# HKU-BAL/MegaGTA

Hardware: AMD Instinct MI355X
Metric: HMM-scored node expansions/sec + SdBG-build Gk-mer/s, k=45, 100Mx150bp (higher is better)
Workload: dtype u32

## Files before the change

### megagta_amd/csrc/device_utils.hpp

```cpp
#pragma once
#include <hip/hip_runtime.h>
#include <cstdint>

namespace mgta {

constexpr int kWave = 64;

__device__ __forceinline__ int lane_id() { return threadIdx.x & 63; }
__device__ __forceinline__ int wave_id() { return threadIdx.x >> 6; }
__device__ __forceinline__ uint64_t lanemask_lt() { return (1ull << lane_id()) - 1ull; }

__device__ __forceinline__ uint32_t wave_incl_scan(uint32_t v) {
    int l = lane_id();
#pragma unroll
    for (int d = 1; d < 64; d <<= 1) {
        uint32_t t = __shfl_up(v, d, 64);
        if (l >= d) v += t;
    }
    return v;
}
__device__ __forceinline__ uint64_t wave_incl_scan64(uint64_t v) {
    int l = lane_id();
#pragma unroll
    for (int d = 1; d < 64; d <<= 1) {
// ... 72 lines not shown
    uint32_t res = scratch[w] + inc - v;
    if (total) *total = scratch[NW];
    return res;
}
template <int NT>
__device__ __forceinline__ uint64_t block_excl_scan64(uint64_t v, uint64_t *scratch, uint64_t *total) {
    constexpr int NW = NT / 64;
    uint64_t inc = wave_incl_scan64(v);
    int w = wave_id(), l = lane_id();
    __syncthreads();
    if (l == 63) scratch[w] = inc;
    __syncthreads();
    if (w == 0) {
        uint64_t x = l < NW ? scratch[l] : 0;
        uint64_t xi = wave_incl_scan64(x);
        if (l < NW) scratch[l] = xi - x;
        if (l == NW - 1) scratch[NW] = xi;
    }
    __syncthreads();
    uint64_t res = scratch[w] + inc - v;
    if (total) *total = scratch[NW];
    return res;
}

constexpr unsigned long long kChainAggregate = 1ull << 62, kChainInclusive = 2ull << 62, kChainValue = (1ull << 62) - 1ull;
constexpr uint32_t kChainSpinLimit = 1u << 19;

__device__ __forceinline__ uint32_t chain_ticket(uint32_t *ticket, uint32_t *s_slot) {
    if (threadIdx.x == 0) *s_slot = atomicAdd(ticket, 1u);
    __syncthreads();
    return wave_uniform(*s_slot);
}

__device__ __forceinline__ uint64_t chain_exclusive(unsigned long long *state, uint32_t tile, uint64_t agg, uint32_t *error) {
    const int lane = lane_id();
    if (tile == 0) {
        if (lane == 0) __hip_atomic_store(&state[0], kChainInclusive | agg, __ATOMIC_RELAXED, __HIP_MEMORY_SCOPE_AGENT);
        return 0;
    }
    if (lane == 0) __hip_atomic_store(&state[tile], kChainAggregate | agg, __ATOMIC_RELAXED, __HIP_MEMORY_SCOPE_AGENT);
    uint64_t excl = 0;
    long long base = (long long)tile - 1;
    uint32_t spins = 0;
    for (;;) {
        const long long t = base - lane;
        const unsigned long long v = t >= 0 ? __hip_atomic_load(&state[t], __ATOMIC_RELAXED, __HIP_MEMORY_SCOPE_AGENT) : kChainInclusive;
        const uint32_t flag = (uint32_t)(v >> 62);
        const uint64_t empty = __ballot(flag == 0), incl = __ballot(flag == 2);
        const int first_incl = incl ? __ffsll((long long)incl) - 1 : 64;
        const uint64_t need = first_incl >= 63 ? ~0ull : ((2ull << first_incl) - 1ull);
        if (empty & need) {
            ++spins;
            if (spins > kChainSpinLimit || ((spins & 255u) == 0 && __hip_atomic_load(error, __ATOMIC_RELAXED, __HIP_MEMORY_SCOPE_AGENT))) {
                if (lane == 0) atomicExch(error, 1u);
                break;
            }
            __builtin_amdgcn_s_sleep(16);
            continue;
        }
        excl += wave_sum64(lane <= first_incl ? (uint64_t)(v & kChainValue) : 0ull);
        if (first_incl < 64) break;
        base -= 64;
    }
    if (lane == 0) __hip_atomic_store(&state[tile], kChainInclusive | ((excl + agg) & kChainValue), __ATOMIC_RELAXED, __HIP_MEMORY_SCOPE_AGENT);
    return excl;
}

}
```

### megagta_amd/csrc/sdbg_build.hip

```cpp
#include <algorithm>
#include <cmath>
#include <cstdlib>
#include <memory>
#include <type_traits>

#include "common.hpp"
#include "device_utils.hpp"
#include "scan.hpp"
#include "segment_split.hpp"

namespace mgta {

constexpr int kDollar = 4;

template <int W>
struct Key {
    uint32_t w[W];
};

template <int W>
__device__ __forceinline__ void shl_bits(uint32_t (&x)[W], int s) {
    if (s == 0) return;
    if (s == 32) {
#pragma unroll
// ... 1648 lines not shown
            uint64_t idx = base + (uint64_t)i * 256 + threadIdx.x;
            if (idx < n && key_prefix<W>(keys[idx], T) != pre && (unsigned long long)idx < found) found = idx;
        }
        if (found != ~0ull) atomicMin(&s_end, found);
        __syncthreads();
        if (s_end != ~0ull) break;
    }
    __syncthreads();
    if (threadIdx.x == 0) big_end[blockIdx.x] = s_end == ~0ull ? n : s_end;
}

constexpr int kEmitThreads = 256;
constexpr int kEmitPerThread = 16;
constexpr int kEmitTile = kEmitThreads * kEmitPerThread;

constexpr int kRunBaseStepLog = 10;
struct RunStarts {
    uint32_t *lo;
    uint64_t *base;
};
__device__ __forceinline__ uint64_t run_full_start(const RunStarts &r, uint64_t s) {
    const uint64_t b = r.base[s >> kRunBaseStepLog];
    return b + (uint32_t)(r.lo[s] - (uint32_t)b);
}
__device__ __forceinline__ uint64_t run_length(const RunStarts &r, uint64_t s, uint64_t m, uint64_t n_items) {
    return s + 1 < m ? (uint64_t)(uint32_t)(r.lo[s + 1] - r.lo[s]) : n_items - run_full_start(r, s);
}

struct EmitChain {
    unsigned long long *state;
    uint32_t *ticket;
    uint32_t *error;
    unsigned long long *total;
};

template <int W, bool TICKET>
__global__ __launch_bounds__(kEmitThreads) void emit_compact_kernel(const Key<W> *keys, uint64_t n, int k, EmitChain chain, uint32_t n_tiles,
                                                                     RunStarts sub_start, uint8_t *sub_info) {
    __shared__ uint32_t s_cnt[kEmitPerThread * (kEmitThreads / 64)];
    __shared__ uint32_t s_scr[kEmitThreads / 64 + 1];
    __shared__ uint32_t s_tile;
    __shared__ unsigned long long s_base;
    const uint32_t tile = TICKET ? chain_ticket(chain.ticket, &s_tile) : blockIdx.x;
    uint64_t base = (uint64_t)tile * kEmitTile;
    const int lane = lane_id(), wv = wave_id();
    uint32_t headbits = 0;
    uint32_t rank_in_wave[kEmitPerThread];
    uint8_t info[kEmitPerThread];
#pragma unroll
    for (int it = 0; it < kEmitPerThread; ++it) {
        uint64_t idx = base + (uint64_t)it * kEmitThreads + threadIdx.x;
        bool head = false;
        info[it] = 0;
        if (idx < n) {
            Key<W> cur = keys[idx];
            if (idx == 0) {
                head = true;
                info[it] = head_info<W>(cur, k, true, true);
            } else
                info[it] = key_info<W>(cur, keys[idx - 1], k, head);
        }
        uint64_t bal = __ballot(head);
        rank_in_wave[it] = (uint32_t)__popcll(bal & lanemask_lt());
        headbits |= (uint32_t)head << it;
        if (lane == 0) s_cnt[it * (kEmitThreads / 64) + wv] = (uint32_t)__popcll(bal);
    }
    __syncthreads();
    uint32_t v = threadIdx.x < kEmitPerThread * (kEmitThreads / 64) ? s_cnt[threadIdx.x] : 0, tile_total = 0;
    uint32_t ex = block_excl_scan<kEmitThreads>(v, s_scr, &tile_total);
    __syncthreads();
    if (threadIdx.x < kEmitPerThread * (kEmitThreads / 64)) s_cnt[threadIdx.x] = ex;
    if (wv == 0) {
        const uint64_t before = chain_exclusive(chain.state, tile, tile_total, chain.error);
        if (lane == 0) {
            s_base = before;
            if (tile + 1 == n_tiles) *chain.total = before + tile_total;
        }
    }
    __syncthreads();
    uint64_t tb = s_base;
#pragma unroll
    for (int it = 0; it < kEmitPerThread; ++it) {
        if ((headbits >> it) & 1u) {
            uint64_t idx = base + (uint64_t)it * kEmitThreads + threadIdx.x;
            uint64_t s = tb + s_cnt[it * (kEmitThreads / 64) + wv] + rank_in_wave[it];
            sub_start.lo[s] = (uint32_t)idx;
            if ((s & ((1u << kRunBaseStepLog) - 1)) == 0) sub_start.base[s >> kRunBaseStepLog] = idx;
            sub_info[s] = info[it];
        }
    }
}

constexpr int kInfoRounds = 8;
constexpr int kInfoTile = kEmitTile * kInfoRounds;
template <bool TICKET>
__global__ __launch_bounds__(kEmitThreads) void emit_compact_info_kernel(const uint8_t *info_in, uint64_t n, EmitChain chain, uint32_t n_tiles,
                                                                          RunStarts sub_start, uint8_t *sub_info) {
    static_assert(kEmitPerThread == 16, "one 16-byte load per lane and round");
    static_assert(kInfoRounds == 8 && kEmitTile <= 65535, "round counts are scanned as 2 x 4 fields of 16 bits");
    __shared__ uint64_t s_scr[kEmitThreads / 64 + 1];
    __shared__ uint32_t s_tile;
    __shared__ unsigned long long s_base;
    __shared__ uint16_t s_off[kEmitTile];
    __shared__ uint8_t s_inf[kEmitTile];
    const uint32_t tile = TICKET ? chain_ticket(chain.ticket, &s_tile) : blockIdx.x;
    const uint64_t base = (uint64_t)tile * kInfoTile;
    const uint32_t mine = threadIdx.x * kEmitPerThread;
    uint4 v[kInfoRounds];
#pragma unroll
    for (int r = 0; r < kInfoRounds; ++r) {
        const uint64_t idx0 = base + (uint64_t)r * kEmitTile + mine;
        v[r] = make_uint4(0, 0, 0, 0);
        if (idx0 < n) v[r] = *reinterpret_cast<const uint4 *>(info_in + idx0);
    }
    uint32_t headbits[kInfoRounds];
    uint64_t packed[2] = {0, 0};
#pragma unroll
    for (int r = 0; r < kInfoRounds; ++r) {
        const uint64_t idx0 = base + (uint64_t)r * kEmitTile + mine;
        const uint32_t left = idx0 < n ? (uint32_t)(n - idx0 < (uint64_t)kEmitPerThread ? n - idx0 : (uint64_t)kEmitPerThread) : 0u;
        const uint32_t wd[4] = {v[r].x, v[r].y, v[r].z, v[r].w};
        uint32_t hb = 0;
#pragma unroll
        for (int b = 0; b < kEmitPerThread; ++b) hb |= (uint32_t)(((wd[b >> 2] >> (8 * (b & 3))) & 7u) != (uint32_t)kInfoNoHead) << b;
        headbits[r] = hb & ((1u << left) - 1u);
        packed[r >> 2] |= (uint64_t)__popc(headbits[r]) << (16 * (r & 3));
    }
    uint64_t ex[2], tot[2];
    ex[0] = block_excl_scan64<kEmitThreads>(packed[0], s_scr, &tot[0]);
    ex[1] = block_excl_scan64<kEmitThreads>(packed[1], s_scr, &tot[1]);
    uint32_t round_total[kInfoRounds], round_first[kInfoRounds], tile_total = 0;
#pragma unroll
    for (int r = 0; r < kInfoRounds; ++r) {
        round_total[r] = (uint32_t)(tot[r >> 2] >> (16 * (r & 3))) & 0xFFFFu;
        round_first[r] = tile_total;
        tile_total += round_total[r];
    }
    if (wave_id() == 0) {
        const uint64_t before = chain_exclusive(chain.state, tile, tile_total, chain.error);
        if (lane_id() == 0) {
            s_base = before;
            if (tile + 1 == n_tiles) *chain.total = before + tile_total;
        }
    }
    uint64_t tb = 0;
#pragma unroll
    for (int r = 0; r < kInfoRounds; ++r) {
        if (round_total[r] == 0) continue;
        const uint32_t wd[4] = {v[r].x, v[r].y, v[r].z, v[r].w};
        uint32_t q = (uint32_t)(ex[r >> 2] >> (16 * (r & 3))) & 0xFFFFu;
#pragma unroll
        for (int b = 0; b < kEmitPerThread; ++b) {
            if ((headbits[r] >> b) & 1u) {
                s_off[q] = (uint16_t)(mine + (uint32_t)b);
                s_inf[q] = (uint8_t)((wd[b >> 2] >> (8 * (b & 3))) & 255u);
                ++q;
            }
        }
        __syncthreads();
        tb = s_base;
        const uint64_t out0 = tb + round_first[r], pos0 = base + (uint64_t)r * kEmitTile;
        for (uint32_t i = threadIdx.x; i < round_total[r]; i += kEmitThreads) {
            const uint64_t s = out0 + i, idx = pos0 + s_off[i];
            sub_start.lo[s] = (uint32_t)idx;
            if ((s & ((1u << kRunBaseStepLog) - 1)) == 0) sub_start.base[s >> kRunBaseStepLog] = idx;
            sub_info[s] = s_inf[i];
        }
        __syncthreads();
    }
}

__global__ __launch_bounds__(256) void emit_check_kernel(const uint32_t *lo, const uint8_t *info, const uint32_t *lo_ref, const uint8_t *info_ref, uint64_t m,
                                                         uint32_t *bad) {
    for (uint64_t s = (uint64_t)blockIdx.x * 256 + threadIdx.x; s < m; s += (uint64_t)gridDim.x * 256) {
        if (lo[s] != lo_ref[s]) atomicAdd(&bad[0], 1u);
        if (info[s] != info_ref[s]) atomicAdd(&bad[1], 1u);
    }
}

template <int W>
__global__ __launch_bounds__(256) void emit_info_range_kernel(const Key<W> *keys, uint64_t n, int k, const uint64_t *start, const uint64_t *end, int stride,
                                                              uint8_t *key_info_out) {
    const uint64_t first = start[(uint64_t)blockIdx.x * stride] & ~kSegInOther;
    uint64_t last = end[(uint64_t)blockIdx.x * stride];
    if (last > n) last = n;
    for (uint64_t i = first + threadIdx.x; i < last; i += 256) {
        const Key<W> cur = keys[i];
        bool head = true;
        const uint8_t info = i == 0 ? head_info<W>(cur, k, true, true) : key_info<W>(cur, keys[i - 1], k, head);
        key_info_out[i] = head ? info : kInfoNoHead;
    }
}

constexpr int kDecideThreads = 256;
constexpr int kDecidePerThread = 4;
constexpr int kDecideTile = kDecideThreads * kDecidePerThread;
constexpr int kDecideHalo = 32;

__device__ __forceinline__ bool run_suppressed(int a, int b, int has_a, int has_b) {
    return (a == kDollar && ((has_b >> b) & 1)) || (b == kDollar && ((has_a >> a) & 1));
}

// ... 53 lines not shown
            ne++;
            nl += count > 254;
            nt += tip;
        }
        rec[s] = r;
    }
    ne = wave_sum(ne); nl = wave_sum(nl); nt = wave_sum(nt);
    if (lane_id() == 0) { s_e[wave_id()] = ne; s_l[wave_id()] = nl; s_t[wave_id()] = nt; }
    __syncthreads();
    if (threadIdx.x == 0) {
        uint32_t e = 0, l = 0, t = 0;
        for (int w = 0; w < kDecideThreads / 64; ++w) { e += s_e[w]; l += s_l[w]; t += s_t[w]; }
        cnt_e[blockIdx.x] = e; cnt_l[blockIdx.x] = l; cnt_t[blockIdx.x] = t;
    }
}

template <int W>
__global__ __launch_bounds__(kDecideThreads) void emit_write_kernel(const Key<W> *keys, RunStarts sub_start, const uint8_t *sub_info, const uint16_t *rec,
                                                                     uint64_t m, uint64_t n_items, const uint64_t *base_e,
                                                                     const uint64_t *base_l, const uint64_t *base_t, int words_per_tip,
                                                                     uint32_t b_lo, uint16_t *out_rec, uint16_t *out_large,
                                                                     uint32_t *out_tips, int64_t *bucket_first ) {
    __shared__ uint64_t s_scr[kDecideThreads / 64 + 1];
    uint64_t s0 = (uint64_t)blockIdx.x * kDecideTile + (uint64_t)threadIdx.x * kDecidePerThread;
    uint16_t r[kDecidePerThread];
    uint64_t packed = 0;
    uint32_t cnts[kDecidePerThread];
    for (int q = 0; q < kDecidePerThread; ++q) {
        uint64_t s = s0 + q;
        r[q] = 0xFFFF; cnts[q] = 0;
        if (s < m) {
            r[q] = rec[s];
            if (r[q] != 0xFFFF) {
                uint64_t run = run_length(sub_start, s, m, n_items);
                cnts[q] = run > 65535 ? 65535u : (uint32_t)run;
                packed += 1ull + ((uint64_t)(cnts[q] > 254) << 20) + ((uint64_t)((r[q] >> 5) & 1) << 40);
            }
        }
    }
    uint64_t ex = block_excl_scan64<kDecideThreads>(packed, s_scr, nullptr);
    uint64_t ie = base_e[blockIdx.x] + (ex & 0xFFFFF), il = base_l[blockIdx.x] + ((ex >> 20) & 0xFFFFF),
             it = base_t[blockIdx.x] + (ex >> 40);
    for (int q = 0; q < kDecidePerThread; ++q) {
        uint64_t s = s0 + q;
        if (s >= m) break;
        const bool is_tip = r[q] != 0xFFFF && ((r[q] >> 5) & 1);
        const bool bucket_head = (sub_info[s] & 128) != 0;
        const uint64_t first_item = (is_tip || bucket_head) ? run_full_start(sub_start, s) : 0;
        if (bucket_head) {
            uint32_t bucket = keys[first_item].w[0] >> 16;
            int64_t *bf = bucket_first + (uint64_t)(bucket - b_lo) * 3;
            bf[0] = (int64_t)ie; bf[1] = (int64_t)il; bf[2] = (int64_t)it;
        }
        if (r[q] != 0xFFFF) {
            out_rec[ie++] = r[q];
            if (cnts[q] > 254) out_large[il++] = (uint16_t)cnts[q];
            if ((r[q] >> 5) & 1) {
                for (int j = 0; j < words_per_tip; ++j) out_tips[it * words_per_tip + j] = keys[first_item].w[j];
                it++;
            }
        }
    }
}

}
#include "sdbg_solid.hpp"
namespace mgta {

static std::vector<Digit> low_digit_plan(int k, int W, int T) {
    std::vector<Digit> plan;
    int pad = 32 * W - 2 * k - 4, top = 32 * W - T;
    if (top > 0) plan.push_back(Digit{0, std::min(4, top)});
    for (int pos = 4 + pad; pos < top; pos += 8) plan.push_back(Digit{pos, std::min(8, top - pos)});
    return plan;
}

template <class T>
static T *pool_get(mgta_ctx *ctx, int slot, uint64_t bytes) {
    if ((int)ctx->pool.size() < S_NUM) ctx->pool.resize(S_NUM);
    DevBuf &b = ctx->pool[slot];
    if (b.bytes < bytes || !b.p) {
        b.release();
        b.alloc(bytes + bytes / 8, &ctx->live_bytes, &ctx->peak_bytes);
    }
    return b.as<T>();
}
static uint64_t pool_bytes(const mgta_ctx *ctx) {
    uint64_t t = 0;
    for (const DevBuf &b : ctx->pool) t += b.bytes;
    return t;
}

struct SortModes {
    int bias = 1, side = 1, fused = 1, wide = 1, emit_fused = 1;
    static SortModes from_env() {
        const char *bias = getenv("MGTA_SORT_BIAS"), *side = getenv("MGTA_SORT_SIDE"), *fused = getenv("MGTA_SORT_FUSED"), *wide = getenv("MGTA_SORT_WIDE");
        const char *emit_fused = getenv("MGTA_EMIT_FUSED");
        return SortModes{bias ? atoi(bias) : 1, side ? atoi(side) : 1, fused ? atoi(fused) : 1, wide ? atoi(wide) : 1, emit_fused ? atoi(emit_fused) : 1};
    }
};

static double avg_segment_len(uint64_t n_items, int p, double prefix_frac) { return (double)n_items / std::max(1.0, std::pow(256.0, p) * prefix_frac); }
static double avg_segment_len_bits(uint64_t n_items, int bits, double prefix_frac) { return (double)n_items / std::max(1.0, std::pow(2.0, bits) * prefix_frac); }
constexpr int kMaxTop = 4;
struct TopPlan {
    int P = 0, skip = 0;
    uint32_t bias = 0;
    double frac = 1.0;
    int width[kMaxTop] = {8, 8, 8, 8};
    int key_bits() const { int t = 0; for (int i = 0; i < P; ++i) t += width[i]; return t; }
    int T() const { return key_bits() + skip; }
    int n_wide() const { int c = 0; for (int i = 0; i < P; ++i) c += width[i] > 8; return c; }
    int max_width() const { int m = 8; for (int i = 0; i < P; ++i) m = std::max(m, width[i]); return m; }
    bool same_digits(const TopPlan &o) const {
        bool same = P == o.P && skip == o.skip && bias == o.bias;
        for (int i = 0; same && i < P; ++i) same = width[i] == o.width[i];
        return same;
    }
    Digit pass_digit(int W, int i) const {
        int below = skip;
        for (int j = 0; j <= i; ++j) below += width[j];
        return Digit{32 * W - below, width[i], bias};
    }
    double avg_segment(uint64_t n_items) const { return avg_segment_len_bits(n_items, key_bits(), frac); }
};
static TopPlan choose_top_plan(const mgta_ctx *ctx, uint64_t n_items, int max_top, double prefix_frac, uint32_t b_lo = 0, uint32_t b_hi = 0,
                               int mode = 0) {
    TopPlan plain;
    plain.frac = prefix_frac;
    if (ctx && ctx->force_full_lsd) return plain;
    while (plain.P < max_top && avg_segment_len(n_items, plain.P, prefix_frac) > (plain.P >= 3 ? 700.0 : 256.0)) ++plain.P;
// ... 713 lines not shown
            sa.side = nullptr;
        }
        S.ms_gen += t_ph.stop();
    }

    Key<W> *sort_keys(const SortJob<W> &job) {
        t_ph.start();
        Key<W> *sorted = device_sort(ctx, job, &log, &sorted_info);
        if (sorted) S.ms_sort += t_ph.stop();
        return sorted;
    }

    int drop_sentinels(Pass &p) {
        if (!p.closed_form || ((k + 1) & 1)) return MGTA_OK;
        unsigned long long n_sent = 0;
        MGTA_HIP_CHECK(hipMemcpy(&n_sent, d_sentinel, 8, hipMemcpyDeviceToHost));
        if (n_sent >= p.n_items) { set_error("internal: %llu sentinel keys among %llu items", n_sent, (unsigned long long)p.n_items); return MGTA_EINTERNAL; }
        p.n_items -= n_sent;
        S.n_items -= (int64_t)n_sent;
        return MGTA_OK;
    }

    int emit(Pass &p, const Key<W> *sorted, Key<W> *scratch_keys) {
        const uint64_t n_items = p.n_items;
        t_ph.start();
        char *scratch = reinterpret_cast<char *>(scratch_keys);
        uint64_t e_tiles = (n_items + kEmitTile - 1) / kEmitTile;
        uint64_t *d_scan_tmp = pool_get<uint64_t>(ctx, S_SCAN_TMP, scan_tmp_elems(std::max<uint64_t>(std::max(n_blocks, e_tiles), n_items / kDecideTile + 1)) * 8);
        if (e_tiles > 0xFFFFFFFFull) { set_error("too many emit tiles"); return MGTA_EUNSUPPORTED; }
        unsigned long long *d_chain = pool_get<unsigned long long>(ctx, S_TILE_BASE, (e_tiles + 4) * 8);
        RunStarts sub_start;
        sub_start.lo = reinterpret_cast<uint32_t *>(scratch);
        uint16_t *rec = reinterpret_cast<uint16_t *>(scratch + n_items * 4);
        uint8_t *info = reinterpret_cast<uint8_t *>(scratch + n_items * 6);
        sub_start.base = reinterpret_cast<uint64_t *>(scratch + ((n_items * 7 + 7) & ~7ull));
        auto compact = [&](const uint8_t *key_info, RunStarts st, uint8_t *st_info, uint64_t *m_out) {
            unsigned long long chain_out[3] = {0, 0, 0};
            const uint64_t tiles = key_info ? (n_items + kInfoTile - 1) / kInfoTile : e_tiles;
            EmitChain chain;
            chain.state = d_chain; chain.total = d_chain + tiles;
            chain.ticket = reinterpret_cast<uint32_t *>(d_chain + tiles + 1); chain.error = reinterpret_cast<uint32_t *>(d_chain + tiles + 2);
            for (int attempt = 0; attempt < 2; ++attempt) {
                MGTA_HIP_CHECK(hipMemsetAsync(d_chain, 0, (tiles + 4) * 8, stream));
                const bool ticket = !(attempt == 0 && !ctx->force_full_lsd);
                const dim3 grid((unsigned)tiles), block(kEmitThreads);
                if (key_info && !ticket)
                    hipLaunchKernelGGL((emit_compact_info_kernel<false>), grid, block, 0, stream, key_info, n_items, chain, (uint32_t)tiles, st, st_info);
                else if (key_info)
                    hipLaunchKernelGGL((emit_compact_info_kernel<true>), grid, block, 0, stream, key_info, n_items, chain, (uint32_t)tiles, st, st_info);
                else if (!ticket)
                    hipLaunchKernelGGL((emit_compact_kernel<W, false>), grid, block, 0, stream, sorted, n_items, k, chain, (uint32_t)tiles, st, st_info);
                else
                    hipLaunchKernelGGL((emit_compact_kernel<W, true>), grid, block, 0, stream, sorted, n_items, k, chain, (uint32_t)tiles, st, st_info);
                MGTA_HIP_CHECK(hipMemcpyAsync(chain_out, d_chain + tiles, 24, hipMemcpyDeviceToHost, stream));
                MGTA_HIP_CHECK(hipStreamSynchronize(stream));
                if ((uint32_t)chain_out[2] == 0) break;
            }
            if ((uint32_t)chain_out[2] != 0) { set_error("internal: chained scan of the emitter timed out"); return MGTA_EINTERNAL; }
            *m_out = chain_out[0];
            return MGTA_OK;
        };
        uint64_t m = 0;
        if (int rc = compact(sorted_info, sub_start, info, &m)) return rc;
        if (sorted_info) {
            ctx->emit_fused_passes++;
            if (modes.emit_fused >= 2) {
                RunStarts ref;
                uint8_t *ref_info = reinterpret_cast<uint8_t *>(rec);
                char *behind = reinterpret_cast<char *>(sub_start.base + (n_items >> kRunBaseStepLog) + 1);
                ref.lo = reinterpret_cast<uint32_t *>(behind);
                ref.base = reinterpret_cast<uint64_t *>(behind + ((n_items * 4 + 7) & ~7ull));
                if ((uint64_t)(reinterpret_cast<char *>(ref.base + (n_items >> kRunBaseStepLog) + 1) - scratch) > p.key_b) {
                    set_error("internal: no room to check the emitter's info bytes");
                    return MGTA_EINTERNAL;
                }
                uint64_t m_ref = 0;
                if (int rc = compact(nullptr, ref, ref_info, &m_ref)) return rc;
                uint32_t *d_bad = reinterpret_cast<uint32_t *>(pool_get<uint64_t>(ctx, S_SMALL, 4096) + 320);
                uint32_t bad[2] = {0, 0};
                MGTA_HIP_CHECK(hipMemsetAsync(d_bad, 0, 8, stream));
                const uint64_t m_min = std::min(m, m_ref);
                if (m_min > 0) {
                    const unsigned grid = (unsigned)std::min<uint64_t>((m_min + 255) / 256, (uint64_t)ctx->num_cus * 16);
                    hipLaunchKernelGGL(emit_check_kernel, dim3(grid), dim3(256), 0, stream, sub_start.lo, info, ref.lo, ref_info, m_min, d_bad);
                }
                MGTA_HIP_CHECK(hipMemcpyAsync(bad, d_bad, 8, hipMemcpyDeviceToHost, stream));
                MGTA_HIP_CHECK(hipStreamSynchronize(stream));
                if (m != m_ref || bad[0] || bad[1]) {
                    set_error("internal: the info bytes of the sort give %llu runs, the keys %llu; %u starts and %u info bytes differ",
                              (unsigned long long)m, (unsigned long long)m_ref, bad[0], bad[1]);
                    return MGTA_EINTERNAL;
                }
            }
        }
        uint64_t d_tiles = (m + kDecideTile - 1) / kDecideTile;
        uint32_t *ce = pool_get<uint32_t>(ctx, S_CNT, d_tiles * 4 * 3), *cl = ce + d_tiles, *ct = cl + d_tiles;
        uint64_t *be = pool_get<uint64_t>(ctx, S_BASE, d_tiles * 8 * 3), *bl = be + d_tiles, *bt = bl + d_tiles;
        p.first = pool_get<int64_t>(ctx, S_FIRST, (uint64_t)MGTA_NUM_BUCKETS * 3 * 8);
        MGTA_HIP_CHECK(hipMemsetAsync(p.first, 0xFF, (uint64_t)p.nb() * 3 * 8, stream));
        hipLaunchKernelGGL(emit_decide_kernel, dim3((unsigned)d_tiles), dim3(kDecideThreads), 0, stream, sub_start, info, m, n_items,
                           rec, ce, cl, ct);
        exclusive_scan_u32(stream, ce, d_tiles, be, d_scan_tmp, d_tot3);
        exclusive_scan_u32(stream, cl, d_tiles, bl, d_scan_tmp, d_tot3 + 1);
        exclusive_scan_u32(stream, ct, d_tiles, bt, d_scan_tmp, d_tot3 + 2);
        uint64_t tot3[3];
        MGTA_HIP_CHECK(hipMemcpyAsync(tot3, d_tot3, 24, hipMemcpyDeviceToHost, stream));
        MGTA_HIP_CHECK(hipStreamSynchronize(stream));
        p.n_edges = tot3[0]; p.n_large = tot3[1]; p.n_tips = tot3[2];
        p.rec = pool_get<uint16_t>(ctx, S_OUT_REC, p.n_edges * 2);
        p.large = pool_get<uint16_t>(ctx, S_OUT_LARGE, p.n_large * 2);
        p.tips = pool_get<uint32_t>(ctx, S_OUT_TIPS, p.n_tips * words_per_tip * 4);
        hipLaunchKernelGGL((emit_write_kernel<W>), dim3((unsigned)d_tiles), dim3(kDecideThreads), 0, stream, sorted, sub_start, info, rec, m,
                           n_items, be, bl, bt, words_per_tip, p.b_lo, p.rec, p.large, p.tips, p.first);
        S.ms_emit += t_ph.stop();
        return MGTA_OK;
    }

    void publish_last(uint32_t lo, uint32_t hi, const void *rec, uint64_t n_rec, const void *tips, uint64_t n_tips, const void *first,
                      const void *large, uint64_t n_large) {
        ctx->last_large = large; ctx->last_n_large = n_large;
        ctx->last_rec = rec; ctx->last_n_rec = n_rec; ctx->last_bucket_lo = lo; ctx->last_bucket_hi = hi;
        ctx->last_tips = tips; ctx->last_n_tips = n_tips; ctx->last_first = first; ctx->last_k = k; ctx->last_words_per_tip = words_per_tip;
    }

    void append_to_stream(const Pass &p) {
        const uint64_t tip_b = words_per_tip * 4;
        auto ensure = [&](DevBuf &buf, uint64_t used, uint64_t add) {
            if (used + add <= buf.bytes) return;
            const double done = (double)(p.b_hi - bucket_begin) / (double)(bucket_end - bucket_begin);
            uint64_t want = (uint64_t)((double)(used + add) / std::max(done, 1e-3) * 1.1) + (1u << 20);
            want = std::max<uint64_t>(want, used + add);
            DevBuf bigger;
            bigger.alloc(want, &ctx->live_bytes, &ctx->peak_bytes);
            if (used) MGTA_HIP_CHECK(hipMemcpyAsync(bigger.p, buf.p, used, hipMemcpyDeviceToDevice, stream));
            MGTA_HIP_CHECK(hipStreamSynchronize(stream));
            buf = std::move(bigger);
        };
        ensure(ctx->acc_rec, ctx->acc_n_rec * 2, p.n_edges * 2);
        ensure(ctx->acc_tips, ctx->acc_n_tips * tip_b, p.n_tips * tip_b);
        if (ctx->acc_has_large) {
            ensure(ctx->acc_large, ctx->acc_n_large * 2, p.n_large * 2);
            if (p.n_large) MGTA_HIP_CHECK(hipMemcpyAsync(ctx->acc_large.as<char>() + ctx->acc_n_large * 2, p.large, p.n_large * 2, hipMemcpyDeviceToDevice, stream));
        }
        if (p.n_edges) MGTA_HIP_CHECK(hipMemcpyAsync(ctx->acc_rec.as<char>() + ctx->acc_n_rec * 2, p.rec, p.n_edges * 2, hipMemcpyDeviceToDevice, stream));
        if (p.n_tips) MGTA_HIP_CHECK(hipMemcpyAsync(ctx->acc_tips.as<char>() + ctx->acc_n_tips * tip_b, p.tips, p.n_tips * tip_b, hipMemcpyDeviceToDevice, stream));
        h_first.resize((size_t)p.nb() * 3);
// ... 189 lines not shown
```

Before: 10.08.

## Fuse emitter decide, scan and write into one chained-scan kernel

Replaces the emit path's three stages (a decide kernel, three exclusive scans, a host readback and sync, then a write kernel) with one kernel. That kernel decides records per tile, publishes counts through two decoupled look-back chains and writes compacted output through shared memory. Output buffers are sized up front from upper bounds (run count, dollar heads counted in the compact kernel, n_items/255), which removes the mid-pass host round trip. It also stores small run counts in the record's high byte so the write kernel can skip run_length lookups. The cost is larger allocations, spin-wait risk with a retry path, and a verification mode that runs both paths.

```diff
diff --git a/megagta_amd/csrc/device_utils.hpp b/megagta_amd/csrc/device_utils.hpp
--- a/megagta_amd/csrc/device_utils.hpp
+++ b/megagta_amd/csrc/device_utils.hpp
@@ -128,13 +128,12 @@
     return wave_uniform(*s_slot);
 }
 
-__device__ __forceinline__ uint64_t chain_exclusive(unsigned long long *state, uint32_t tile, uint64_t agg, uint32_t *error) {
+__device__ __forceinline__ void chain_publish(unsigned long long *state, uint32_t tile, uint64_t agg) {
+    if (lane_id() == 0) __hip_atomic_store(&state[tile], (tile == 0 ? kChainInclusive : kChainAggregate) | agg, __ATOMIC_RELAXED, __HIP_MEMORY_SCOPE_AGENT);
+}
+__device__ __forceinline__ uint64_t chain_look_back(unsigned long long *state, uint32_t tile, uint64_t agg, uint32_t *error) {
     const int lane = lane_id();
-    if (tile == 0) {
-        if (lane == 0) __hip_atomic_store(&state[0], kChainInclusive | agg, __ATOMIC_RELAXED, __HIP_MEMORY_SCOPE_AGENT);
-        return 0;
-    }
-    if (lane == 0) __hip_atomic_store(&state[tile], kChainAggregate | agg, __ATOMIC_RELAXED, __HIP_MEMORY_SCOPE_AGENT);
+    if (tile == 0) return 0;
     uint64_t excl = 0;
     long long base = (long long)tile - 1;
     uint32_t spins = 0;
@@ -161,5 +160,9 @@
     if (lane == 0) __hip_atomic_store(&state[tile], kChainInclusive | ((excl + agg) & kChainValue), __ATOMIC_RELAXED, __HIP_MEMORY_SCOPE_AGENT);
     return excl;
 }
+__device__ __forceinline__ uint64_t chain_exclusive(unsigned long long *state, uint32_t tile, uint64_t agg, uint32_t *error) {
+    chain_publish(state, tile, agg);
+    return chain_look_back(state, tile, agg, error);
+}
 
 }
diff --git a/megagta_amd/csrc/sdbg_build.hip b/megagta_amd/csrc/sdbg_build.hip
--- a/megagta_amd/csrc/sdbg_build.hip
+++ b/megagta_amd/csrc/sdbg_build.hip
@@ -1704,19 +1704,29 @@
     uint32_t *ticket;
     uint32_t *error;
     unsigned long long *total;
+    unsigned long long *dollar;
 };
+constexpr int kDollarSlots = 64;
+__device__ __forceinline__ void count_dollar_heads(const EmitChain &chain, uint32_t tile, uint32_t mine, uint32_t *s_sum) {
+    if (threadIdx.x == 0) *s_sum = 0;
+    __syncthreads();
+    mine = wave_sum(mine);
+    if (lane_id() == 0 && mine) atomicAdd(s_sum, mine);
+    __syncthreads();
+    if (threadIdx.x == 0 && *s_sum) atomicAdd(&chain.dollar[tile % kDollarSlots], (unsigned long long)*s_sum);
+}
 
 template <int W, bool TICKET>
 __global__ __launch_bounds__(kEmitThreads) void emit_compact_kernel(const Key<W> *keys, uint64_t n, int k, EmitChain chain, uint32_t n_tiles,
                                                                      RunStarts sub_start, uint8_t *sub_info) {
     __shared__ uint32_t s_cnt[kEmitPerThread * (kEmitThreads / 64)];
     __shared__ uint32_t s_scr[kEmitThreads / 64 + 1];
-    __shared__ uint32_t s_tile;
+    __shared__ uint32_t s_tile, s_dollar;
     __shared__ unsigned long long s_base;
     const uint32_t tile = TICKET ? chain_ticket(chain.ticket, &s_tile) : blockIdx.x;
     uint64_t base = (uint64_t)tile * kEmitTile;
     const int lane = lane_id(), wv = wave_id();
-    uint32_t headbits = 0;
+    uint32_t headbits = 0, n_dollar = 0;
     uint32_t rank_in_wave[kEmitPerThread];
     uint8_t info[kEmitPerThread];
 #pragma unroll
@@ -1759,8 +1769,10 @@
             sub_start.lo[s] = (uint32_t)idx;
             if ((s & ((1u << kRunBaseStepLog) - 1)) == 0) sub_start.base[s >> kRunBaseStepLog] = idx;
             sub_info[s] = info[it];
-        }
-    }
+            n_dollar += (info[it] & 7) == kDollar;
+        }
+    }
+    count_dollar_heads(chain, tile, n_dollar, &s_dollar);
 }
 
 constexpr int kInfoRounds = 8;
@@ -1771,7 +1783,7 @@
     static_assert(kEmitPerThread == 16, "one 16-byte load per lane and round");
     static_assert(kInfoRounds == 8 && kEmitTile <= 65535, "round counts are scanned as 2 x 4 fields of 16 bits");
     __shared__ uint64_t s_scr[kEmitThreads / 64 + 1];
-    __shared__ uint32_t s_tile;
+    __shared__ uint32_t s_tile, s_dollar;
     __shared__ unsigned long long s_base;
     __shared__ uint16_t s_off[kEmitTile];
     __shared__ uint8_t s_inf[kEmitTile];
@@ -1816,6 +1828,7 @@
         }
     }
     uint64_t tb = 0;
+    uint32_t n_dollar = 0;
 #pragma unroll
     for (int r = 0; r < kInfoRounds; ++r) {
         if (round_total[r] == 0) continue;
@@ -1836,10 +1849,13 @@
             const uint64_t s = out0 + i, idx = pos0 + s_off[i];
             sub_start.lo[s] = (uint32_t)idx;
             if ((s & ((1u << kRunBaseStepLog) - 1)) == 0) sub_start.base[s >> kRunBaseStepLog] = idx;
-            sub_info[s] = s_inf[i];
+            const uint8_t inf = s_inf[i];
+            sub_info[s] = inf;
+            n_dollar += (inf & 7) == kDollar;
         }
         __syncthreads();
     }
+    count_dollar_heads(chain, tile, n_dollar, &s_dollar);
 }
 
 __global__ __launch_bounds__(256) void emit_check_kernel(const uint32_t *lo, const uint8_t *info, const uint32_t *lo_ref, const uint8_t *info_ref, uint64_t m,
@@ -1959,8 +1975,11 @@
         if (s < m) {
             r[q] = rec[s];
             if (r[q] != 0xFFFF) {
-                uint64_t run = run_length(sub_start, s, m, n_items);
-                cnts[q] = run > 65535 ? 65535u : (uint32_t)run;
+                cnts[q] = r[q] >> 8;
+                if (cnts[q] == 255) {
+                    uint64_t run = run_length(sub_start, s, m, n_items);
+                    cnts[q] = run > 65535 ? 65535u : (uint32_t)run;
+                }
                 packed += 1ull + ((uint64_t)(cnts[q] > 254) << 20) + ((uint64_t)((r[q] >> 5) & 1) << 40);
             }
         }
@@ -1990,6 +2009,243 @@
     }
 }
 
+constexpr int kChainRounds = 8;
+constexpr int kChainTile = kDecideTile * kChainRounds;
+constexpr int kChainSlots = kChainRounds * kDecidePerThread * (kDecideThreads / 64);
+constexpr int kChainTipBits = 34;
+static_assert(kChainTipBits < 62 && kChainTile < (1 << 20), "the second chain's value, the packed tile counts");
+struct DecideChain {
+    unsigned long long *state_e, *state_lt;
+    uint32_t *ticket, *error;
+    uint64_t *totals;
+};
+
+template <int W, bool TICKET>
+__global__ __launch_bounds__(kDecideThreads, 6) void emit_decide_write_kernel(const Key<W> *keys, RunStarts sub_start, const uint8_t *sub_info, uint64_t m,
+                                                                            uint64_t n_items, DecideChain chain, uint32_t n_tiles, int words_per_tip,
+                                                                            uint32_t b_lo, uint16_t *out_rec, uint16_t *out_large, uint32_t *out_tips,
+                                                                            int64_t *bucket_first ) {
+    constexpr int NW = kDecideThreads / 64, NQ = kDecidePerThread;
+    constexpr int kChunks = (kChainTile + 2 * kDecideHalo) / 16, kChunkIters = (kChunks + kDecideThreads - 1) / kDecideThreads;
+    static_assert(NQ == 4 && kDecideHalo % 16 == 0 && kChainSlots <= kDecideThreads, "four decisions per word; 16-byte loads; one scan");
+    __shared__ uint4 s_info4[kChunks];
+    __shared__ uint16_t s_out[kChainTile];
+    __shared__ uint64_t s_cnt[kChainSlots];
+    __shared__ uint64_t s_scr[NW + 1];
+    __shared__ uint32_t s_tile;
+    __shared__ unsigned long long s_base[2];
+    const uint8_t *s_info = reinterpret_cast<const uint8_t *>(s_info4);
+    const uint32_t tile = TICKET ? chain_ticket(chain.ticket, &s_tile) : blockIdx.x;
+    const uint64_t t0 = (uint64_t)tile * kChainTile;
+    const uint32_t tid = threadIdx.x;
+    const int lane = lane_id(), wv = wave_id();
+    const uint8_t *info_t = sub_info + t0;
+    const uint32_t *lo_t = sub_start.lo + t0;
+    const int m_l = (int)(m - t0 < (1ull << 30) ? m - t0 : (1ull << 30));
+    const uint32_t n_t = (uint32_t)(m_l < kChainTile + 1 ? m_l : kChainTile + 1);
+    const int w_lo = tile ? -kDecideHalo : 0, w_hi = m_l < kChainTile + kDecideHalo ? m_l : kChainTile + kDecideHalo;
+
+    uint4 iv[kChunkIters];
+#pragma unroll
+    for (int j = 0; j < kChunkIters; ++j) {
+        const uint32_t c = (uint32_t)j * kDecideThreads + tid;
+        const int at = 16 * (int)c - kDecideHalo;
+        iv[j] = make_uint4(0, 0, 0, 0);
+        if (c < (uint32_t)kChunks && at >= w_lo && at < m_l) iv[j] = *reinterpret_cast<const uint4 *>(info_t + at);
+    }
+    uint32_t cnt2[kChainRounds][NQ / 2];
+    const bool owns_last = n_t <= (uint32_t)kChainTile && ((n_t - 1) & (kDecideThreads - 1)) == tid;
+    uint32_t last_len = 0;
+#pragma unroll
+    for (int half = 0; half < 2; ++half) {
+        uint32_t lo0[kChainRounds / 2][NQ], lo1[kChainRounds / 2][NQ];
+#pragma unroll
+        for (int r = 0; r < kChainRounds / 2; ++r)
+#pragma unroll
+            for (int q = 0; q < NQ; ++q) {
+                const uint32_t idx = (uint32_t)(((half * (kChainRounds / 2) + r) * NQ + q) * kDecideThreads) + tid;
+                lo0[r][q] = lo_t[idx < n_t - 1 ? idx : n_t - 1];
+                lo1[r][q] = lo_t[idx + 1 < n_t - 1 ? idx + 1 : n_t - 1];
+            }
+        if (half == 0) {
+#pragma unroll
+            for (int j = 0; j < kChunkIters; ++j) {
+                const uint32_t c = (uint32_t)j * kDecideThreads + tid;
+                if (c < (uint32_t)kChunks) s_info4[c] = iv[j];
+            }
+            if (owns_last) {
+                const uint64_t rest = n_items - run_full_start(sub_start, t0 + n_t - 1);
+                last_len = rest > 65535 ? 65535u : (uint32_t)rest;
+            }
+        }
+        __builtin_amdgcn_sched_barrier(0);
+#pragma unroll
+        for (int r = 0; r < kChainRounds / 2; ++r) {
+            const int rr = half * (kChainRounds / 2) + r;
+            cnt2[rr][0] = cnt2[rr][1] = 0;
+#pragma unroll
+            for (int q = 0; q < NQ; ++q) {
+                uint32_t len = lo1[r][q] - lo0[r][q];
+                if (owns_last && (uint32_t)(rr * NQ + q) == (n_t - 1) / kDecideThreads) len = last_len;
+                cnt2[rr][q >> 1] |= (len > 65535u ? 65535u : len) << (16 * (q & 1));
+            }
+            asm volatile("" : "+v"(cnt2[rr][0]), "+v"(cnt2[rr][1]));
+        }
+        __builtin_amdgcn_sched_barrier(0);
+    }
+    __syncthreads();
+
+    auto info_at = [&](int j) -> int { return (j >= w_lo && j < w_hi) ? (int)s_info[j + kDecideHalo] : (int)info_t[j]; };
+    uint32_t dec[kChainRounds];
+#pragma unroll
+    for (int r = 0; r < kChainRounds; ++r) dec[r] = ~0u;
+#pragma unroll 1
+    for (int r = 0; r < kChainRounds; ++r) {
+        uint32_t c01 = 0, c23 = 0, dr = 0;
+#pragma unroll
+        for (int rr = 0; rr < kChainRounds; ++rr)
+            if (rr == r) { c01 = cnt2[rr][0]; c23 = cnt2[rr][1]; }
+#pragma unroll
+        for (int q = 0; q < NQ; ++q) {
+            const int s = (r * NQ + q) * kDecideThreads + (int)tid;
+            const uint32_t count = ((q & 2 ? c23 : c01) >> (16 * (q & 1))) & 0xFFFFu;
+            uint32_t d = 0xFFu;
+            if (s < m_l) {
+                const int inf = info_at(s);
+                const int a = inf & 7, b = (inf >> 3) & 7;
+                int has_a = 0, has_b = 0;
+                auto collect = [&](int xi) {
+                    const int xa = xi & 7, xb = (xi >> 3) & 7;
+                    if (xa != kDollar && xb != kDollar) { has_a |= 1 << xa; has_b |= 1 << xb; }
+                };
+                collect(inf);
+                bool front_b_solid = false, front_b_dollar = false;
+                int gs = s;
+                for (int gi = inf; !(gi & 64);) {
+                    --gs; gi = info_at(gs); collect(gi);
+                    if (((gi >> 3) & 7) == b) { if ((gi & 7) != kDollar) front_b_solid = true; else front_b_dollar = true; }
+                }
+                int ge = s + 1;
+                while (ge < m_l) {
+                    const int xi = info_at(ge);
+                    if (xi & 64) break;
+                    collect(xi);
+                    ++ge;
+                }
+                if (!run_suppressed(a, b, has_a, has_b)) {
+                    const bool seen_b = front_b_solid || (front_b_dollar && !((has_b >> b) & 1));
+                    const int w = (b == kDollar) ? 0 : (seen_b ? b + 5 : b + 1);
+                    int last = 0;
+                    if (a != kDollar) {
+                        bool later = false;
+                        for (int x = s + 1; x < ge; ++x) {
+                            const int xi = info_at(x), xa = xi & 7, xb = (xi >> 3) & 7;
+                            if (xa == a && (xb != kDollar || !((has_a >> a) & 1))) later = true;
+                        }
+                        last = later ? 0 : 1;
+                    }
+                    d = (uint32_t)(w | (last << 4) | ((a == kDollar) << 5));
+                }
+            }
+            dr |= d << (8 * q);
+            const bool em = d != 0xFFu;
+            const uint64_t bal_e = __ballot(em), bal_l = __ballot(em && count > 254u), bal_t = __ballot(em && (d & 32u));
+            if (lane == 0)
+                s_cnt[(r * NQ + q) * NW + wv] = (uint64_t)__popcll(bal_e) | (uint64_t)__popcll(bal_l) << 20 | (uint64_t)__popcll(bal_t) << 40;
+        }
+#pragma unroll
+        for (int rr = 0; rr < kChainRounds; ++rr)
+            if (rr == r) dec[rr] = dr;
+    }
+    __syncthreads();
+
+    uint64_t tot = 0;
+    const uint64_t ex = block_excl_scan64<kDecideThreads>(tid < (uint32_t)kChainSlots ? s_cnt[tid] : 0ull, s_scr, &tot);
+    if (tid < (uint32_t)kChainSlots) s_cnt[tid] = ex;
+    const uint32_t te = (uint32_t)tot & 0xFFFFFu, tl = (uint32_t)(tot >> 20) & 0xFFFFFu, tt = (uint32_t)(tot >> 40);
+    const uint64_t agg_lt = (uint64_t)tl << kChainTipBits | tt;
+    if (wv == 0) chain_publish(chain.state_e, tile, te);
+    if (wv == 1) chain_publish(chain.state_lt, tile, agg_lt);
+    __syncthreads();
+
+#pragma unroll
+    for (int r = 0; r < kChainRounds; ++r)
+#pragma unroll
+        for (int q = 0; q < NQ; ++q) {
+            const uint32_t d = (dec[r] >> (8 * q)) & 0xFFu, count = (cnt2[r][q >> 1] >> (16 * (q & 1))) & 0xFFFFu;
+            const bool em = d != 0xFFu;
+            const uint64_t bal_e = __ballot(em);
+            if (em) {
+                const uint32_t at = ((uint32_t)s_cnt[(r * NQ + q) * NW + wv] & 0xFFFFFu) + (uint32_t)__popcll(bal_e & lanemask_lt());
+                s_out[at] = (uint16_t)(d | (count > 255u ? 255u : count) << 8);
+            }
+        }
+    if (wv == 0) {
+        const uint64_t before = chain_look_back(chain.state_e, tile, te, chain.error);
+        if (lane == 0) {
+            s_base[0] = before;
+            if (tile + 1 == n_tiles) chain.totals[0] = before + te;
+        }
+    }
+    if (wv == 1) {
+        const uint64_t before = chain_look_back(chain.state_lt, tile, agg_lt, chain.error);
+        if (lane == 0) {
+            s_base[1] = before;
+            if (tile + 1 == n_tiles) { chain.totals[1] = (before >> kChainTipBits) + tl; chain.totals[2] = (before & ((1ull << kChainTipBits) - 1ull)) + tt; }
+        }
+    }
+    __syncthreads();
+    const uint64_t be = s_base[0], bl = s_base[1] >> kChainTipBits, bt = s_base[1] & ((1ull << kChainTipBits) - 1ull);
+
+    {
+        uint32_t head = (uint32_t)((8u - (uint32_t)(be & 7u)) & 7u);
+        if (head > te) head = te;
+        const uint32_t n8 = (te - head) >> 3, tail0 = head + (n8 << 3);
+        if (tid < head) out_rec[be + tid] = s_out[tid];
+        for (uint32_t c = tid; c < n8; c += kDecideThreads) {
+            const uint32_t i = head + (c << 3);
+            uint4 v;
+            v.x = (uint32_t)s_out[i] | (uint32_t)s_out[i + 1] << 16; v.y = (uint32_t)s_out[i + 2] | (uint32_t)s_out[i + 3] << 16;
+            v.z = (uint32_t)s_out[i + 4] | (uint32_t)s_out[i + 5] << 16; v.w = (uint32_t)s_out[i + 6] | (uint32_t)s_out[i + 7] << 16;
+            *reinterpret_cast<uint4 *>(out_rec + be + i) = v;
+        }
+        if (tail0 + tid < te) out_rec[be + tail0 + tid] = s_out[tail0 + tid];
+    }
+
+#pragma unroll
+    for (int r = 0; r < kChainRounds; ++r)
+#pragma unroll
+        for (int q = 0; q < NQ; ++q) {
+            const int k0 = (r * NQ + q) * kDecideThreads;
+            const uint32_t d = (dec[r] >> (8 * q)) & 0xFFu, count = (cnt2[r][q >> 1] >> (16 * (q & 1))) & 0xFFFFu;
+            const bool em = d != 0xFFu, large = em && count > 254u, tip = em && (d & 32u);
+            const bool bucket_head = (int)tid < m_l - k0 && (s_info[kDecideHalo + k0 + tid] & 128) != 0;
+            if (__ballot(large || tip || bucket_head) == 0) continue;
+            const uint64_t bal_e = __ballot(em), bal_l = __ballot(large), bal_t = __ballot(tip), lt = lanemask_lt();
+            const uint64_t x = s_cnt[(r * NQ + q) * NW + wv];
+            const uint64_t ie = be + ((uint32_t)x & 0xFFFFFu) + (uint32_t)__popcll(bal_e & lt);
+            const uint64_t il = bl + ((uint32_t)(x >> 20) & 0xFFFFFu) + (uint32_t)__popcll(bal_l & lt);
+            const uint64_t it = bt + (uint32_t)(x >> 40) + (uint32_t)__popcll(bal_t & lt);
+            if (large) out_large[il] = (uint16_t)count;
+            if (tip || bucket_head) {
+                const uint64_t first_item = run_full_start(sub_start, t0 + k0 + tid);
+                if (bucket_head) {
+                    const uint32_t bucket = keys[first_item].w[0] >> 16;
+                    int64_t *bf = bucket_first + (uint64_t)(bucket - b_lo) * 3;
+                    bf[0] = (int64_t)ie; bf[1] = (int64_t)il; bf[2] = (int64_t)it;
+                }
+                if (tip)
+                    for (int j = 0; j < words_per_tip; ++j) out_tips[it * words_per_tip + j] = keys[first_item].w[j];
+            }
+        }
+}
+
+template <class T>
+__global__ __launch_bounds__(256) void emit_equal_kernel(const T *a, const T *b, uint64_t n, uint32_t *bad) {
+    for (uint64_t i = (uint64_t)blockIdx.x * 256 + threadIdx.x; i < n; i += (uint64_t)gridDim.x * 256)
+        if (a[i] != b[i]) atomicAdd(bad, 1u);
+}
+
 }
 #include "sdbg_solid.hpp"
 namespace mgta {
@@ -2019,11 +2275,12 @@
 }
 
 struct SortModes {
-    int bias = 1, side = 1, fused = 1, wide = 1, emit_fused = 1;
+    int bias = 1, side = 1, fused = 1, wide = 1, emit_fused = 1, emit_chain = 1;
     static SortModes from_env() {
         const char *bias = getenv("MGTA_SORT_BIAS"), *side = getenv("MGTA_SORT_SIDE"), *fused = getenv("MGTA_SORT_FUSED"), *wide = getenv("MGTA_SORT_WIDE");
-        const char *emit_fused = getenv("MGTA_EMIT_FUSED");
-        return SortModes{bias ? atoi(bias) : 1, side ? atoi(side) : 1, fused ? atoi(fused) : 1, wide ? atoi(wide) : 1, emit_fused ? atoi(emit_fused) : 1};
+        const char *emit_fused = getenv("MGTA_EMIT_FUSED"), *emit_chain = getenv("MGTA_EMIT_CHAIN");
+        return SortModes{bias ? atoi(bias) : 1, side ? atoi(side) : 1, fused ? atoi(fused) : 1, wide ? atoi(wide) : 1, emit_fused ? atoi(emit_fused) : 1,
+                         emit_chain ? atoi(emit_chain) : 1};
     }
 };
 
@@ -2803,16 +3060,20 @@
         RunStarts sub_start;
         sub_start.lo = reinterpret_cast<uint32_t *>(scratch);
         uint16_t *rec = reinterpret_cast<uint16_t *>(scratch + n_items * 4);
-        uint8_t *info = reinterpret_cast<uint8_t *>(scratch + n_items * 6);
-        sub_start.base = reinterpret_cast<uint64_t *>(scratch + ((n_items * 7 + 7) & ~7ull));
-        auto compact = [&](const uint8_t *key_info, RunStarts st, uint8_t *st_info, uint64_t *m_out) {
+        const uint64_t info_at = (n_items * 6 + 15) & ~15ull;
+        uint8_t *info = reinterpret_cast<uint8_t *>(scratch + info_at);
+        sub_start.base = reinterpret_cast<uint64_t *>(scratch + ((info_at + n_items + 15) & ~15ull));
+        unsigned long long *d_dollar = reinterpret_cast<unsigned long long *>(pool_get<uint64_t>(ctx, S_SMALL, 4096) + 64);
+        auto compact = [&](const uint8_t *key_info, RunStarts st, uint8_t *st_info, uint64_t *m_out, uint64_t *n_dollar_out) {
             unsigned long long chain_out[3] = {0, 0, 0};
+            unsigned long long dollar[kDollarSlots];
             const uint64_t tiles = key_info ? (n_items + kInfoTile - 1) / kInfoTile : e_tiles;
             EmitChain chain;
-            chain.state = d_chain; chain.total = d_chain + tiles;
+            chain.state = d_chain; chain.total = d_chain + tiles; chain.dollar = d_dollar;
             chain.ticket = reinterpret_cast<uint32_t *>(d_chain + tiles + 1); chain.error = reinterpret_cast<uint32_t *>(d_chain + tiles + 2);
             for (int attempt = 0; attempt < 2; ++attempt) {
                 MGTA_HIP_CHECK(hipMemsetAsync(d_chain, 0, (tiles + 4) * 8, stream));
+                MGTA_HIP_CHECK(hipMemsetAsync(d_dollar, 0, sizeof(dollar), stream));
                 const bool ticket = !(attempt == 0 && !ctx->force_full_lsd);
                 const dim3 grid((unsigned)tiles), block(kEmitThreads);
                 if (key_info && !ticket)
@@ -2824,15 +3085,18 @@
                 else
                     hipLaunchKernelGGL((emit_compact_kernel<W, true>), grid, block, 0, stream, sorted, n_items, k, chain, (uint32_t)tiles, st, st_info);
                 MGTA_HIP_CHECK(hipMemcpyAsync(chain_out, d_chain + tiles, 24, hipMemcpyDeviceToHost, stream));
+                MGTA_HIP_CHECK(hipMemcpyAsync(dollar, d_dollar, sizeof(dollar), hipMemcpyDeviceToHost, stream));
                 MGTA_HIP_CHECK(hipStreamSynchronize(stream));
                 if ((uint32_t)chain_out[2] == 0) break;
             }
             if ((uint32_t)chain_out[2] != 0) { set_error("internal: chained scan of the emitter timed out"); return MGTA_EINTERNAL; }
             *m_out = chain_out[0];
+            *n_dollar_out = 0;
+            for (unsigned long long d : dollar) *n_dollar_out += d;
             return MGTA_OK;
         };
-        uint64_t m = 0;
-        if (int rc = compact(sorted_info, sub_start, info, &m)) return rc;
+        uint64_t m = 0, n_dollar = 0;
+        if (int rc = compact(sorted_info, sub_start, info, &m, &n_dollar)) return rc;
         if (sorted_info) {
             ctx->emit_fused_passes++;
             if (modes.emit_fused >= 2) {
@@ -2845,8 +3109,10 @@
                     set_error("internal: no room to check the emitter's info bytes");
                     return MGTA_EINTERNAL;
                 }
-                uint64_t m_ref = 0;
-                if (int rc = compact(nullptr, ref, ref_info, &m_ref)) return rc;
+                uint64_t m_ref = 0, n_dollar_ref = 0;
+                if (int rc = compact(nullptr, ref, ref_info, &m_ref, &n_dollar_ref)) return rc;
+                if (n_dollar_ref != n_dollar) { set_error("internal: the info bytes of the sort give %llu runs with a = $, the keys %llu",
+                                                          (unsigned long long)n_dollar, (unsigned long long)n_dollar_ref); return MGTA_EINTERNAL; }
                 uint32_t *d_bad = reinterpret_cast<uint32_t *>(pool_get<uint64_t>(ctx, S_SMALL, 4096) + 320);
                 uint32_t bad[2] = {0, 0};
                 MGTA_HIP_CHECK(hipMemsetAsync(d_bad, 0, 8, stream));
@@ -2864,25 +3130,104 @@
                 }
             }
         }
-        uint64_t d_tiles = (m + kDecideTile - 1) / kDecideTile;
-        uint32_t *ce = pool_get<uint32_t>(ctx, S_CNT, d_tiles * 4 * 3), *cl = ce + d_tiles, *ct = cl + d_tiles;
-        uint64_t *be = pool_get<uint64_t>(ctx, S_BASE, d_tiles * 8 * 3), *bl = be + d_tiles, *bt = bl + d_tiles;
-        p.first = pool_get<int64_t>(ctx, S_FIRST, (uint64_t)MGTA_NUM_BUCKETS * 3 * 8);
-        MGTA_HIP_CHECK(hipMemsetAsync(p.first, 0xFF, (uint64_t)p.nb() * 3 * 8, stream));
-        hipLaunchKernelGGL(emit_decide_kernel, dim3((unsigned)d_tiles), dim3(kDecideThreads), 0, stream, sub_start, info, m, n_items,
-                           rec, ce, cl, ct);
-        exclusive_scan_u32(stream, ce, d_tiles, be, d_scan_tmp, d_tot3);
-        exclusive_scan_u32(stream, cl, d_tiles, bl, d_scan_tmp, d_tot3 + 1);
-        exclusive_scan_u32(stream, ct, d_tiles, bt, d_scan_tmp, d_tot3 + 2);
-        uint64_t tot3[3];
-        MGTA_HIP_CHECK(hipMemcpyAsync(tot3, d_tot3, 24, hipMemcpyDeviceToHost, stream));
-        MGTA_HIP_CHECK(hipStreamSynchronize(stream));
-        p.n_edges = tot3[0]; p.n_large = tot3[1]; p.n_tips = tot3[2];
-        p.rec = pool_get<uint16_t>(ctx, S_OUT_REC, p.n_edges * 2);
-        p.large = pool_get<uint16_t>(ctx, S_OUT_LARGE, p.n_large * 2);
-        p.tips = pool_get<uint32_t>(ctx, S_OUT_TIPS, p.n_tips * words_per_tip * 4);
-        hipLaunchKernelGGL((emit_write_kernel<W>), dim3((unsigned)d_tiles), dim3(kDecideThreads), 0, stream, sorted, sub_start, info, rec, m,
-                           n_items, be, bl, bt, words_per_tip, p.b_lo, p.rec, p.large, p.tips, p.first);
+        struct Out { uint16_t *rec = nullptr, *large = nullptr; uint32_t *tips = nullptr; int64_t *first = nullptr; uint64_t tot[3] = {0, 0, 0}; };
+        DevBuf t_rec, t_large, t_tips, t_first;
+        auto room = [&](bool pooled, int slot, DevBuf &tmp, uint64_t bytes) -> void * {
+            if (pooled) return pool_get<char>(ctx, slot, bytes);
+            tmp.alloc(bytes, &ctx->live_bytes, &ctx->peak_bytes);
+            return tmp.p;
+        };
+        const uint64_t first_b = (uint64_t)MGTA_NUM_BUCKETS * 3 * 8;
+        auto three_steps = [&](bool pooled, Out &o) -> int {
+            const uint64_t d_tiles = (m + kDecideTile - 1) / kDecideTile;
+            uint32_t *ce = pool_get<uint32_t>(ctx, S_CNT, d_tiles * 4 * 3), *cl = ce + d_tiles, *ct = cl + d_tiles;
+            uint64_t *be = pool_get<uint64_t>(ctx, S_BASE, d_tiles * 8 * 3), *bl = be + d_tiles, *bt = bl + d_tiles;
+            o.first = static_cast<int64_t *>(room(pooled, S_FIRST, t_first, first_b));
+            MGTA_HIP_CHECK(hipMemsetAsync(o.first, 0xFF, (uint64_t)p.nb() * 3 * 8, stream));
+            hipLaunchKernelGGL(emit_decide_kernel, dim3((unsigned)d_tiles), dim3(kDecideThreads), 0, stream, sub_start, info, m, n_items,
+                               rec, ce, cl, ct);
+            exclusive_scan_u32(stream, ce, d_tiles, be, d_scan_tmp, d_tot3);
+            exclusive_scan_u32(stream, cl, d_tiles, bl, d_scan_tmp, d_tot3 + 1);
+            exclusive_scan_u32(stream, ct, d_tiles, bt, d_scan_tmp, d_tot3 + 2);
+            MGTA_HIP_CHECK(hipMemcpyAsync(o.tot, d_tot3, 24, hipMemcpyDeviceToHost, stream));
+            MGTA_HIP_CHECK(hipStreamSynchronize(stream));
+            o.rec = static_cast<uint16_t *>(room(pooled, S_OUT_REC, t_rec, o.tot[0] * 2));
+            o.large = static_cast<uint16_t *>(room(pooled, S_OUT_LARGE, t_large, o.tot[1] * 2));
+            o.tips = static_cast<uint32_t *>(room(pooled, S_OUT_TIPS, t_tips, o.tot[2] * words_per_tip * 4));
+            hipLaunchKernelGGL((emit_write_kernel<W>), dim3((unsigned)d_tiles), dim3(kDecideThreads), 0, stream, sorted, sub_start, info, rec, m,
+                               n_items, be, bl, bt, words_per_tip, p.b_lo, o.rec, o.large, o.tips, o.first);
+            return MGTA_OK;
+        };
+        auto chained = [&](Out &o) -> int {
+            if ((m >> kChainTipBits) != 0 || ((n_items / 255) >> (62 - kChainTipBits)) != 0) {
+                set_error("too many runs (%llu) or keys (%llu) for the emitter's chained scan", (unsigned long long)m, (unsigned long long)n_items);
+                return MGTA_EUNSUPPORTED;
+            }
+            const uint64_t tiles = (m + kChainTile - 1) / kChainTile;
+            DecideChain dc;
+            dc.state_e = d_chain; dc.state_lt = d_chain + tiles; dc.totals = d_tot3;
+            dc.ticket = reinterpret_cast<uint32_t *>(d_chain + 2 * tiles); dc.error = reinterpret_cast<uint32_t *>(d_chain + 2 * tiles + 1);
+            o.rec = pool_get<uint16_t>(ctx, S_OUT_REC, m * 2);
+            o.large = pool_get<uint16_t>(ctx, S_OUT_LARGE, (n_items / 255 + 1) * 2);
+            o.tips = pool_get<uint32_t>(ctx, S_OUT_TIPS, n_dollar * words_per_tip * 4);
+            o.first = pool_get<int64_t>(ctx, S_FIRST, first_b);
+            unsigned long long err = 0;
+            for (int attempt = 0; attempt < 2; ++attempt) {
+                MGTA_HIP_CHECK(hipMemsetAsync(d_chain, 0, (2 * tiles + 2) * 8, stream));
+                MGTA_HIP_CHECK(hipMemsetAsync(d_tot3, 0, 24, stream));
+                MGTA_HIP_CHECK(hipMemsetAsync(o.first, 0xFF, (uint64_t)p.nb() * 3 * 8, stream));
+                const dim3 grid((unsigned)tiles), block(kDecideThreads);
+                if (attempt == 0 && !ctx->force_full_lsd)
+                    hipLaunchKernelGGL((emit_decide_write_kernel<W, false>), grid, block, 0, stream, sorted, sub_start, info, m, n_items, dc, (uint32_t)tiles,
+                                       words_per_tip, p.b_lo, o.rec, o.large, o.tips, o.first);
+                else
+                    hipLaunchKernelGGL((emit_decide_write_kernel<W, true>), grid, block, 0, stream, sorted, sub_start, info, m, n_items, dc, (uint32_t)tiles,
+                                       words_per_tip, p.b_lo, o.rec, o.large, o.tips, o.first);
+                MGTA_HIP_CHECK(hipMemcpyAsync(o.tot, d_tot3, 24, hipMemcpyDeviceToHost, stream));
+                MGTA_HIP_CHECK(hipMemcpyAsync(&err, d_chain + 2 * tiles + 1, 8, hipMemcpyDeviceToHost, stream));
+                MGTA_HIP_CHECK(hipStreamSynchronize(stream));
+                if ((uint32_t)err == 0) break;
+            }
+            if ((uint32_t)err != 0) { set_error("internal: chained scan of the emitter's records timed out"); return MGTA_EINTERNAL; }
+            if (o.tot[0] > m || o.tot[1] > n_items / 255 + 1 || o.tot[2] > n_dollar) {
+                set_error("internal: the emitter wrote %llu records, %llu large counts and %llu tips into room for %llu, %llu and %llu", (unsigned long long)o.tot[0],
+                          (unsigned long long)o.tot[1], (unsigned long long)o.tot[2], (unsigned long long)m, (unsigned long long)(n_items / 255 + 1), (unsigned long long)n_dollar);
+                return MGTA_EINTERNAL;
+            }
+            return MGTA_OK;
+        };
+        Out out, ref;
+        if (modes.emit_chain <= 0) {
+            if (int rc = three_steps(true, out)) return rc;
+        } else {
+            if (modes.emit_chain >= 2)
+                if (int rc = three_steps(false, ref)) return rc;
+            if (int rc = chained(out)) return rc;
+        }
+        if (modes.emit_chain >= 2) {
+            uint32_t *d_bad = reinterpret_cast<uint32_t *>(pool_get<uint64_t>(ctx, S_SMALL, 4096) + 320);
+            uint32_t bad[4] = {0, 0, 0, 0};
+            MGTA_HIP_CHECK(hipMemsetAsync(d_bad, 0, 16, stream));
+            const bool same_totals = out.tot[0] == ref.tot[0] && out.tot[1] == ref.tot[1] && out.tot[2] == ref.tot[2];
+            auto grid_of = [&](uint64_t n) { return dim3((unsigned)std::min<uint64_t>((n + 255) / 256, (uint64_t)ctx->num_cus * 16)); };
+            if (same_totals) {
+                const uint64_t n_tw = out.tot[2] * words_per_tip, n_f = (uint64_t)p.nb() * 3;
+                if (out.tot[0]) hipLaunchKernelGGL((emit_equal_kernel<uint16_t>), grid_of(out.tot[0]), dim3(256), 0, stream, out.rec, ref.rec, out.tot[0], d_bad);
+                if (out.tot[1]) hipLaunchKernelGGL((emit_equal_kernel<uint16_t>), grid_of(out.tot[1]), dim3(256), 0, stream, out.large, ref.large, out.tot[1], d_bad + 1);
+                if (n_tw) hipLaunchKernelGGL((emit_equal_kernel<uint32_t>), grid_of(n_tw), dim3(256), 0, stream, out.tips, ref.tips, n_tw, d_bad + 2);
+                hipLaunchKernelGGL((emit_equal_kernel<int64_t>), grid_of(n_f), dim3(256), 0, stream, out.first, ref.first, n_f, d_bad + 3);
+            }
+            MGTA_HIP_CHECK(hipMemcpyAsync(bad, d_bad, 16, hipMemcpyDeviceToHost, stream));
+            MGTA_HIP_CHECK(hipStreamSynchronize(stream));
+            if (!same_totals || bad[0] || bad[1] || bad[2] || bad[3]) {
+                set_error("internal: one emit kernel gives %llu records, %llu large, %llu tips, the three steps %llu, %llu, %llu; %u records, %u large counts, "
+                          "%u tip words and %u bucket entries differ", (unsigned long long)out.tot[0], (unsigned long long)out.tot[1], (unsigned long long)out.tot[2],
+                          (unsigned long long)ref.tot[0], (unsigned long long)ref.tot[1], (unsigned long long)ref.tot[2], bad[0], bad[1], bad[2], bad[3]);
+                return MGTA_EINTERNAL;
+            }
+        }
+        p.rec = out.rec; p.large = out.large; p.tips = out.tips; p.first = out.first;
+        p.n_edges = out.tot[0]; p.n_large = out.tot[1]; p.n_tips = out.tot[2];
         S.ms_emit += t_ph.stop();
         return MGTA_OK;
     }
```

After: 10.32 (median of 6 runs). 1.02x the previous value.
